# Blosc/c-blosc

Measured on NVIDIA H100. Metric: compress+decompress GB/s, higher is better.
Workload: dtype u8

## Files before the change

c-blosc_b200/csrc/dev_lz4.cuh:

```cuda
#pragma once
#include "dev_common.cuh"

#define LZ4_MFLIMIT 12
#define LZ4_LASTLITERALS 5
#define LZ4_TABLE_BYTES 16384
#define LZ4_TAB17_BYTES (8192 + 512)
#define LZ4_TAB17_MINLEN 65547
#define LZ4_TAB17_MAXLEN 131072

template <bool U16>
DEV u32 lz4_hash_at(const u8* __restrict__ s, int pos) {
  if (U16) return (ld_u32(s + pos) * 2654435761u) >> (32 - 13);
  const u64 seq = (u64)ld_u32(s + pos) | ((u64)s[pos + 4] << 32);
  return (u32)(((seq << 24) * 889523592379ull) >> (64 - 12));
}

#define LZ4_SCALAR_PROBES 4

DEV long long lz4_probe_offset(int it, int accel) {
  if (it == 0) return 0;
  const long long m = it - 1;
  const long long c = m >> 6;
  return 1 + m * accel + 32 * c * (c - 1) + c * (m - 64 * c);
}

struct StreamBase {
  const u8* s;
  const u32* s32;
  int sal;
  const uint4* s128;
  int sal16;
};
DEV StreamBase make_stream_base(const u8* s) {
  StreamBase b;
  b.s = s;
  b.s32 = (const u32*)((uintptr_t)s & ~(uintptr_t)3);
  b.sal = (int)((uintptr_t)s & 3u);
  b.s128 = (const uint4*)((uintptr_t)s & ~(uintptr_t)15);
  b.sal16 = (int)((uintptr_t)s & 15u);
  return b;
}
DEV void ldp_win12(const StreamBase& sb, int p, u32& b0, u32& b1, u32& b2) {
#ifdef SIMT_EMU
  memcpy(&b0, sb.s + p, 4); memcpy(&b1, sb.s + p + 4, 4); memcpy(&b2, sb.s + p + 8, 4);
#else
  const int q = p + sb.sal;
  const u32* w = sb.s32 + (q >> 2);
  const u32 sh = (u32)(q & 3) * 8u;
  const u32 w0 = __ldg(w), w1 = __ldg(w + 1), w2 = __ldg(w + 2), w3 = __ldg(w + 3);
  b0 = __funnelshift_r(w0, w1, sh); b1 = __funnelshift_r(w1, w2, sh); b2 = __funnelshift_r(w2, w3, sh);
#endif
}
DEV void ldp_raw12(const StreamBase& sb, int p, u32& r0, u32& r1, u32& r2, u32& r3) {
#ifdef SIMT_EMU
  memcpy(&r0, sb.s + p, 4); memcpy(&r1, sb.s + p + 4, 4); memcpy(&r2, sb.s + p + 8, 4); r3 = 0;
#else
  const u32* w = sb.s32 + ((p + sb.sal) >> 2);
  r0 = __ldg(w); r1 = __ldg(w + 1); r2 = __ldg(w + 2); r3 = __ldg(w + 3);
#endif
}
DEV void ldp_take12(const StreamBase& sb, int p, u32 r0, u32 r1, u32 r2, u32 r3, u32& b0, u32& b1, u32& b2) {
#ifdef SIMT_EMU
  (void)sb; (void)p; (void)r3; b0 = r0; b1 = r1; b2 = r2;
#else
  const u32 sh = (u32)((p + sb.sal) & 3) * 8u;
  b0 = __funnelshift_r(r0, r1, sh); b1 = __funnelshift_r(r1, r2, sh); b2 = __funnelshift_r(r2, r3, sh);
#endif
}
DEV void ldp_win8(const StreamBase& sb, int p, u32& b0, u32& b1) {
#ifdef SIMT_EMU
  memcpy(&b0, sb.s + p, 4); memcpy(&b1, sb.s + p + 4, 4);
#else
  const int q = p + sb.sal;
  const u32* w = sb.s32 + (q >> 2);
  const u32 sh = (u32)(q & 3) * 8u;
  const u32 w0 = __ldg(w), w1 = __ldg(w + 1), w2 = __ldg(w + 2);
  b0 = __funnelshift_r(w0, w1, sh); b1 = __funnelshift_r(w1, w2, sh);
#endif
}

DEV void ldp_raw20(const StreamBase& sb, int p, u32 (&r)[5]) {
#ifdef SIMT_EMU
  memcpy(&r[0], sb.s + p, 16); r[4] = sb.s[p + 16];
#else
  const u32* w = sb.s32 + ((p + sb.sal) >> 2);
  r[0] = __ldg(w); r[1] = __ldg(w + 1); r[2] = __ldg(w + 2); r[3] = __ldg(w + 3); r[4] = __ldg(w + 4);
#endif
}
DEV void ldp_take17(const StreamBase& sb, int p, const u32 (&r)[5], u32& a0, u32& a1, u32& a2, u32& a3, u32& a4b) {
#ifdef SIMT_EMU
  (void)sb; (void)p; a0 = r[0]; a1 = r[1]; a2 = r[2]; a3 = r[3]; a4b = r[4] & 0xffu;
#else
  const u32 sh = (u32)((p + sb.sal) & 3) * 8u;
  a0 = __funnelshift_r(r[0], r[1], sh); a1 = __funnelshift_r(r[1], r[2], sh);
  a2 = __funnelshift_r(r[2], r[3], sh); a3 = __funnelshift_r(r[3], r[4], sh);
  a4b = (r[4] >> sh) & 0xffu;
#endif
}
DEV void ldp_gather17(const StreamBase& sb, int p, u32& c0, u32& c1, u32& c2, u32& c3, u32& c4b) {
#ifdef SIMT_EMU
  memcpy(&c0, sb.s + p, 4); memcpy(&c1, sb.s + p + 4, 4); memcpy(&c2, sb.s + p + 8, 4); memcpy(&c3, sb.s + p + 12, 4);
  c4b = sb.s[p + 16];
#else
  const int q = p + sb.sal16;
  const uint4* w = sb.s128 + (q >> 4);
  const uint4 v0 = __ldg(w), v1 = __ldg(w + 1);
  const bool k1 = (q & 4) != 0, k2 = (q & 8) != 0;
  const u32 sh = (u32)(q & 3) * 8u;
  const u32 t0 = k1 ? v0.y : v0.x, t1 = k1 ? v0.z : v0.y, t2 = k1 ? v0.w : v0.z, t3 = k1 ? v1.x : v0.w;
  const u32 t4 = k1 ? v1.y : v1.x, t5 = k1 ? v1.z : v1.y, t6 = k1 ? v1.w : v1.z;
  const u32 u0 = k2 ? t2 : t0, u1 = k2 ? t3 : t1, u2 = k2 ? t4 : t2, u3 = k2 ? t5 : t3, u4 = k2 ? t6 : t4;
  c0 = __funnelshift_r(u0, u1, sh); c1 = __funnelshift_r(u1, u2, sh);
  c2 = __funnelshift_r(u2, u3, sh); c3 = __funnelshift_r(u3, u4, sh);
  c4b = (u4 >> sh) & 0xffu;
#endif
}

DEV void lz4d_prefetch(const u8* base, int p, int end) {
#ifndef SIMT_EMU
  if (p < end) asm volatile("prefetch.global.L1 [%0];" :: "l"(base + p));
#else
  (void)base; (void)p; (void)end;
#endif
}

DEV u32 ldp_win4(const StreamBase& sb, int p) {
#ifdef SIMT_EMU
  u32 b0; memcpy(&b0, sb.s + p, 4); return b0;
#else
  const int q = p + sb.sal;
  const u32* w = sb.s32 + (q >> 2);
  return __funnelshift_r(__ldg(w), __ldg(w + 1), (u32)(q & 3) * 8u);
#endif
}

template <bool U16>
DEV u32 lz4_hash_seq(u32 lo, u32 b4) {
  if (U16) return (lo * 2654435761u) >> (32 - 13);
  const u64 seq = (u64)lo | ((u64)(b4 & 0xffu) << 32);
  return (u32)(((seq << 24) * 889523592379ull) >> (64 - 12));
}

DEV int lz4_count_tail(const StreamBase& sb, const u8* __restrict__ s, int p, int q, int limit, int n) {
  if (p + 136 <= n) {
    const int lane = lane_id();
    const u32 x = ldp_win4(sb, p + 4 * lane) ^ ldp_win4(sb, q + 4 * lane);
    const unsigned full = __ballot_sync(FULLMASK, x == 0u);
    if (full != FULLMASK) {
      const int fl = __ffs((int)~full) - 1;
      return fl * 4 + eq_bytes32(__shfl_sync(FULLMASK, x, fl));
    }
    return 128 + warp_count_match(s, p + 128, q + 128, limit);
  }
  return warp_count_match(s, p, q, limit);
}

DEV int lz4_catch_up(const u8* __restrict__ s, int ip, int match, int anchor, int back) {
  const int lane = lane_id();
  for (;;) {
    const int a = ip - 1 - back - lane, b = match - 1 - back - lane;
    const bool ok = a >= anchor && b >= 0 && s[a] == s[b];
    const unsigned m = __ballot_sync(FULLMASK, ok);
    const int step = m == FULLMASK ? 32 : __ffs((int)~m) - 1;
    back += step;
    if (step < 32) return back;
  }
}

#ifdef SIMT_EMU
static long long g_dbg_lz4t_sessions = 0, g_dbg_lz4t_seqs = 0, g_dbg_lz4t_stale = 0, g_dbg_lz4t_x[6];
enum {
  LZ4T_S_HIT0,
  LZ4T_S_STALE = 4,
  LZ4T_S_MISS4,
  LZ4T_S_LIT,
  LZ4T_S_CAPPED,
  LZ4T_S_LONG,
  LZ4T_S_HUGE,
  LZ4T_S_N
};
static long long g_dbg_lz4t_s[LZ4T_S_N];
enum {
  LZ4T_W_WINDOWS,
  LZ4T_W_ELEMS,
  LZ4T_W_STALE0, LZ4T_W_STALEJ,
  LZ4T_W_FWD,
  LZ4T_W_CROSS,
  LZ4T_W_MISS0, LZ4T_W_MISSJ,
  LZ4T_W_LONG0, LZ4T_W_LONGJ,
  LZ4T_W_HUGE,
  LZ4T_W_END, LZ4T_W_CAP, LZ4T_W_TILE,
  LZ4T_W_FULL,
  LZ4T_W_N
};
static long long g_dbg_lz4t_w[LZ4T_W_N];
#define LZ4T_DBG(x) do { if (lane_id() == 0) (x)++; } while (0)
#define LZ4T_DBGN(x, v) do { if (lane_id() == 0) (x) += (v); } while (0)
#else
#define LZ4T_DBG(x) do {} while (0)
#define LZ4T_DBGN(x, v) do {} while (0)
#endif
#ifndef LZ4T_TILES
#define LZ4T_TILES 12
#endif
#ifndef LZ4T_AHEAD
#define LZ4T_AHEAD 8
#endif
#ifndef LZ4T_NAP
#define LZ4T_NAP 128
#endif
#define LZ4T_RING (32 * LZ4T_TILES)
#define LZ4T_BAR_IDLE(i) (1 + (i))
#define LZ4T_BAR_GO(i) (4 + (i))
#define LZ4T_QUIT 1
#define LZ4T_STOP 0x7fffffff
#define LZ4T_END 0xffffffffu
#define LZ4T_LONG 13
#define LZ4T_HSHIFT 19
#define LZ4T_BACKCAP 7
#define LZ4T_W 16
static_assert(LZ4T_TILES % 3 == 0 && LZ4T_AHEAD >= 1 && LZ4T_AHEAD < LZ4T_TILES && LZ4T_RING > 15 + 255 + 4, "team ring layout");
static_assert(2 * LZ4T_W <= 32, "window layout");
#define LZ4T_PREFETCH 512

enum {
  LZ4C_TOTAL,
  LZ4C_START,
  LZ4C_SESSION,
  LZ4C_FULLWAIT,
  LZ4C_REPROBE,
  LZ4C_SEARCH,
  LZ4C_SESSIONS, LZ4C_SEQS, LZ4C_CHAIN_SEQS,
  LZ4C_PREP_BUSY,
  LZ4C_PREP_OWN,
  LZ4C_PREP_GATHER,
  LZ4C_PREP_TILES,
  LZ4C_SMID, LZ4C_SUBP,
  LZ4C_STALE,
  LZ4C_N = 16
};
enum {
  LZ4C_WINDOWS = LZ4C_N, LZ4C_W_STALE, LZ4C_W_MISS, LZ4C_W_LONG, LZ4C_W_END, LZ4C_W_CAP, LZ4C_W_TILE,
  LZ4C_NREC
};
#ifdef B2_LZ4_CYCLES
#define LZ4C_MAXSTREAMS 16384
__device__ unsigned long long g_lz4_cycles[LZ4C_MAXSTREAMS][LZ4C_NREC];
#define LZ4C_T(t) const long long t = clock64()
#define LZ4C_TW(t) const long long t = TEAM ? clock64() : 0ll
#define LZ4C_ADD(k, v) do { if (lane_id() == 0) atomicAdd(&tm->cyc[k], (unsigned long long)(v)); } while (0)
#define LZ4C_SPAN(k, t) LZ4C_ADD(k, clock64() - (t))
#else
#define LZ4C_T(t) do {} while (0)
#define LZ4C_TW(t) do {} while (0)
#define LZ4C_ADD(k, v) do {} while (0)
#define LZ4C_SPAN(k, t) do {} while (0)
#endif

struct Lz4Team {
  uint2 vd[LZ4T_RING];
  int rdy[LZ4T_TILES];
  const u8* s;
  int n;
  int u16;
  int wt;
  int gen;
  int cmd;
  int sub[4];
  int slot;
  u32 seen[8192 / 32];
#ifdef B2_LZ4_CYCLES
  unsigned long long cyc[LZ4C_NREC];
#endif
};
#define LZ4T_SMEM_BYTES ((int)sizeof(Lz4Team))

DEV int lz4t_ld_i32(const int* p) { return *(const volatile int*)p; }
DEV void lz4t_st_i32(int* p, int v) { *(volatile int*)p = v; }

template <bool U16>
DEV void lz4_team_prepare_tile(Lz4Team* tm, const void* tabmem, const u8* s, int n, int tile) {
  const int lane = lane_id();
  const int w0 = 32 * tile, p = w0 + lane;
  const int e = (tile % LZ4T_TILES) * 32 + lane;
  if (w0 + 31 + 24 > n) { tm->vd[e] = make_uint2(0u, LZ4T_END); return; }
  const StreamBase sb = make_stream_base(s);
  u32 r[5], a0, a1, a2, a3, a4, c0, c1, c2, c3, c4;
  LZ4C_T(c_t0);
  ldp_raw20(sb, p, r);
  ldp_take17(sb, p, r, a0, a1, a2, a3, a4);
  const u32 h = lz4_hash_seq<U16>(a0, a1);
  const int snap = U16 ? (int)((const volatile u16*)tabmem)[h] : (int)((const volatile u32*)tabmem)[h];
  u32 vx = h << LZ4T_HSHIFT, sn = LZ4T_END;
  if ((unsigned)snap < (unsigned)p) {
    LZ4C_T(c_t1);
    LZ4C_ADD(LZ4C_PREP_OWN, c_t1 - c_t0);
    ldp_gather17(sb, snap, c0, c1, c2, c3, c4);
    const u32 x1 = a1 ^ c1, x2 = a2 ^ c2, x3 = a3 ^ c3;
    u32 m;
    if (x1) m = (u32)(__ffs((int)x1) - 1) >> 3;
    else if (x2) m = 4u + ((u32)(__ffs((int)x2) - 1) >> 3);
    else if (x3) m = 8u + ((u32)(__ffs((int)x3) - 1) >> 3);
    else m = a4 != c4 ? 12u : (u32)LZ4T_LONG;
    const bool hit = (U16 || snap + 65535 >= p) && c0 == a0;
    u32 bk = 0;
    if (hit) {
      if (snap >= 8) {
        u32 p0, p1, q0, q1;
        ldp_win8(sb, p - 8, p0, p1);
        ldp_win8(sb, snap - 8, q0, q1);
        const u32 y1 = p1 ^ q1, z0 = (u32)__clz((int)(p0 ^ q0)) >> 3;
        bk = y1 ? (u32)__clz((int)y1) >> 3 : 4u + (z0 < 3u ? z0 : 3u);
      } else {
        while (bk < (u32)snap && s[p - 1 - (int)bk] == s[snap - 1 - (int)bk]) bk++;
      }
    }
    vx |= (hit ? 1u : 0u) | (m << 2) | (bk << 8);
    sn = (u32)snap;
    LZ4C_SPAN(LZ4C_PREP_GATHER, c_t1);
  }
  tm->vd[e] = make_uint2(vx, sn);
}

DEV void lz4_team_preparer(Lz4Team* tm, const void* tabmem, int i) {
  for (;;) {
    bar_sync(LZ4T_BAR_GO(i), 64);
    if (lz4t_ld_i32(&tm->cmd) == LZ4T_QUIT) return;
    const u8* s = *(const u8* const volatile*)&tm->s;
    const int n = lz4t_ld_i32(&tm->n), u16 = lz4t_ld_i32(&tm->u16);
    for (int tile = i;; tile += 3) {
      int w;
      for (;;) {
        w = __shfl_sync(FULLMASK, lz4t_ld_i32(&tm->wt), 0);
        if (w == LZ4T_STOP) break;
        if (tile < w) tile = w + (i + 3 - w % 3) % 3;
        if (tile <= w + LZ4T_AHEAD) break;
        __nanosleep(LZ4T_NAP);
      }
      if (w == LZ4T_STOP) break;
      LZ4C_T(c_go);
      lz4d_prefetch(s, 32 * tile + LZ4T_PREFETCH + lane_id(), n);
      if (u16) lz4_team_prepare_tile<true>(tm, tabmem, s, n, tile);
      else lz4_team_prepare_tile<false>(tm, tabmem, s, n, tile);
      __syncwarp();
      if (lane_id() == 0) { __threadfence_block(); lz4t_st_i32(&tm->rdy[tile % LZ4T_TILES], tile + 1); }
      LZ4C_SPAN(LZ4C_PREP_BUSY, c_go);
      LZ4C_ADD(LZ4C_PREP_TILES, 1);
    }
    __syncwarp();
    bar_arrive(LZ4T_BAR_IDLE(i), 64);
  }
}

DEV void lz4t_reach(Lz4Team* tm, int ip, int& wt, int& vt) {
  const int lo = (ip - 2) >> 5, hi = ip >> 5;
  if (lo > wt + LZ4T_AHEAD) LZ4T_DBG(g_dbg_lz4t_x[2]);
  if (lo != wt) { wt = lo; lz4t_st_i32(&tm->wt, lo); }
  for (int t = vt + 1 > lo ? vt + 1 : lo; t <= hi; t++) {
    const int* r = &tm->rdy[t % LZ4T_TILES];
    if (lz4t_ld_i32(r) != t + 1) {
      LZ4T_DBG(g_dbg_lz4t_x[5]);
      do { __syncwarp(); } while (__any_sync(FULLMASK, lz4t_ld_i32(r) != t + 1));
    }
  }
  if (hi > vt) vt = hi;
}

DEV void lz4t_extend(Lz4Team* tm, int wt, int& vt) {
  const int t = vt + 1 + lane_id();
  const bool ready = t <= wt + LZ4T_AHEAD && lz4t_ld_i32(&tm->rdy[t % LZ4T_TILES]) == t + 1;
  vt += __ffs((int)~__ballot_sync(FULLMASK, ready)) - 1;
}

template <bool U16>
DEV bool lz4t_search(Lz4Team* tm, smem_addr_t vda, void* tabmem, const StreamBase& sb, int n, int anchor, int accel,
                     int& twt, int& tvt, u32& pk, u32& snap, int& ip, bool& hit, int& match, int& back, int& lit,
                     bool& have_mc, int& mc_carry) {
  u16* tab16 = (u16*)tabmem;
  u32* tab32 = (u32*)tabmem;
  const int mfl1 = n - LZ4_MFLIMIT + 1;
  ip = anchor + 1;
  int it = 0, pos = ip;
  for (;; it++) {
    if (it == LZ4_SCALAR_PROBES) { LZ4T_DBG(g_dbg_lz4t_s[LZ4T_S_MISS4]); lit = it; return false; }
    pos = ip + (it ? 1 + (it - 1) * accel : 0);
    if (ip + 1 + it * accel > mfl1) { lit = it; return false; }
    if ((pos >> 5) > tvt) lz4t_reach(tm, pos, twt, tvt);
    u32 qk, qs;
    smem_ld_u32x2(vda, ((u32)pos % (u32)LZ4T_RING) << 3, qk, qs);
    const u32 h = qk >> LZ4T_HSHIFT;
    const int cand = U16 ? (int)tab16[h] : (int)tab32[h];
    __syncwarp();
    if (cand != (int)qs) { LZ4T_DBG(g_dbg_lz4t_s[LZ4T_S_STALE]); lit = it; return false; }
    if (U16) tab16[h] = (u16)pos; else tab32[h] = (u32)pos;
    if (qk & 1u) { pk = qk; snap = qs; break; }
  }
  LZ4T_DBG(g_dbg_lz4t_s[LZ4T_S_HIT0 + it]);
  const int vb = (int)((pk >> 8) & 7u), dist = pos - anchor;
  const int bq = vb < dist ? vb : dist;
  int m = (int)((pk >> 2) & 15u);
  if (m == LZ4T_LONG) {
    LZ4T_DBG(g_dbg_lz4t_s[LZ4T_S_LONG]);
    m = LZ4T_LONG + lz4_count_tail(sb, sb.s, pos + 4 + LZ4T_LONG, (int)snap + 4 + LZ4T_LONG, n - LZ4_LASTLITERALS, n);
  }
  if (bq == dist && bq + m < 15 + 255) {
    const int mc = bq + m;
    snap -= (u32)bq;
    pk = 1u | ((u32)(mc < LZ4T_LONG ? mc : LZ4T_LONG) << 2);
    ip = anchor;
    LZ4C_ADD(LZ4C_SEQS, 1);
    LZ4C_ADD(LZ4C_CHAIN_SEQS, ~0ull);
    return true;
  }
  hit = true; ip = pos; match = (int)snap;
  have_mc = true; mc_carry = m;
  back = bq;
  if (vb == LZ4T_BACKCAP && dist > LZ4T_BACKCAP) {
    LZ4T_DBG(g_dbg_lz4t_s[LZ4T_S_CAPPED]);
    back = lz4_catch_up(sb.s, pos, (int)snap, anchor, LZ4T_BACKCAP);
  } else if (bq != dist) LZ4T_DBG(g_dbg_lz4t_s[LZ4T_S_LIT]);
  else LZ4T_DBG(g_dbg_lz4t_s[LZ4T_S_HUGE]);
  lit = pos - back - anchor;
  return false;
}

template <bool U16, bool PACK, bool TEAM>
DEV int lz4_encode_stream(const u8* __restrict__ s, const int n, u8* __restrict__ d, const int cap,
                          const int accel, void* tabmem, int* need_out, Lz4Team* tm) {
  const int lane = lane_id();
  const StreamBase sb = make_stream_base(s);
  u16* tab16 = (u16*)tabmem;
  u32* tab32 = (u32*)tabmem;
  u32* tabhi = (u32*)((u8*)tabmem + 8192);
#define LZ4_TGET(h) (U16 ? (int)tab16[h] : PACK ? ((int)tab16[h] | (int)(((tabhi[(h) >> 5] >> ((h) & 31u)) & 1u) << 16)) : (int)tab32[h])
#define LZ4_TPUT(h, v) do { if (U16) tab16[h] = (u16)(v); else if (PACK) { tab16[h] = (u16)(v); const u32 m_ = 1u << ((h) & 31u); \
                            if ((v) & 0x10000) atomicOr(&tabhi[(h) >> 5], m_); else atomicAnd(&tabhi[(h) >> 5], ~m_); } \
                            else tab32[h] = (u32)(v); } while (0)

  for (int i = lane; i < (PACK ? LZ4_TAB17_BYTES : LZ4_TABLE_BYTES) / 4; i += 32) tab32[i] = 0;
  __syncwarp();

  const bool limited = (long long)cap < (long long)n + n / 255 + 16;
  const int olimit = cap;
  const int mfl1 = n - LZ4_MFLIMIT + 1;
  const int matchlimit = n - LZ4_LASTLITERALS;
  int ip = 1, anchor = 0, op = 0;
  int need = 0;
#define LZ4_LIMIT(v) do { const int v_ = (v); if (v_ > need) need = v_; if (limited && v_ > olimit) return 0; } while (0)

  int w0 = -(1 << 30);
  u32 wq0 = 0, wq1 = 0, wq2 = 0, wh = 0;
  int pb = -(1 << 30);
  u32 pq0 = 0, pq1 = 0, pq2 = 0, pq3 = 0;
  int nrec = 0, recop = 0;
  u32 rec = 0;
  int twt = 0, tvt = -1;
#define LZ4_FLUSH_CHECKED() do { if (nrec) { LZ4_LIMIT(op + (1 + LZ4_LASTLITERALS)); } LZ4_FLUSH(); } while (0)
#define LZ4_FLUSH() do { if (lane < nrec) { d[recop] = (u8)rec; d[recop + 1] = (u8)(rec >> 8); d[recop + 2] = (u8)(rec >> 16); \
                                             if ((rec & 15u) == 15u) d[recop + 3] = (u8)(rec >> 24); } nrec = 0; } while (0)

  if (n >= LZ4_MFLIMIT + 1) {
    bool post = false;
    for (;;) {
      int match = 0, lit = 0, back = 0;
      u32 ipn = 0, cn = 0;
      bool have_next = false, hit = false, imm = false, have_mc = false;
      int mc_carry = 0;

      bool scalar_post = post;
      if constexpr (TEAM) if (post && ip + 64 <= n) {
        scalar_post = false;
        bool finished = false;
        LZ4T_DBG(g_dbg_lz4t_sessions);
        LZ4C_T(c_s0);
        LZ4C_ADD(LZ4C_SESSIONS, 1);
        if ((ip - 2) >> 5 <= twt + LZ4T_AHEAD) LZ4T_DBG(g_dbg_lz4t_x[3]);
        lz4t_reach(tm, ip, twt, tvt);
        __syncwarp();
        LZ4C_SPAN(LZ4C_START, c_s0);
        LZ4C_T(c_s1);
        const smem_addr_t vda = smem_addr(tm->vd);
        u32 e = (u32)ip % (u32)LZ4T_RING;
        bool given = false;
        u32 gpk = 0, gsnap = 0;
        for (;;) {
          if (nrec > 32 - LZ4T_W) {
#ifdef SIMT_EMU
            if (limited && op + 1 + LZ4_LASTLITERALS > olimit) LZ4T_DBG(g_dbg_lz4t_w[LZ4T_W_FULL]);
#endif
            LZ4_FLUSH_CHECKED();
          }
          lz4t_extend(tm, twt, tvt);
          int cnt = 0, q = ip, why;
          u32 ee = e, pk, snap;
          if (given) { pk = gpk; snap = gsnap; } else smem_ld_u32x2(vda, ee << 3, pk, snap);
          int jq = 0;
          u32 je = 0, jpk = 0, jsnap = 0;
          for (;;) {
            if (lane == cnt) { jq = q; je = ee; jpk = pk; jsnap = snap; }
            cnt++;
            const u32 step = ((pk >> 2) & 15u) + 4u;
            u32 en = ee + step;
            if (en >= (u32)LZ4T_RING) en -= (u32)LZ4T_RING;
            u32 npk, nsnap;
            smem_ld_u32x2(vda, en << 3, npk, nsnap);
            if (!(pk & 1u)) { why = LZ4C_W_MISS; break; }
            if (step == LZ4T_LONG + 4u) { why = LZ4C_W_LONG; break; }
            q += (int)step; ee = en;
            if (cnt == LZ4T_W) { why = LZ4C_W_CAP; break; }
            if (q + 64 > n) { why = LZ4C_W_END; break; }
            if ((q >> 5) > tvt) { why = LZ4C_W_TILE; break; }
            pk = npk; snap = nsnap;
          }
          u32 jh2 = 0;
          if (lane < cnt) jh2 = smem_ld_u32(vda, (je >= 2u ? je - 2u : je - 2u + LZ4T_RING) << 3) >> LZ4T_HSHIFT;
          const int el = lane >> 1;
          const bool odd = (lane & 1) != 0;
          const u32 sh2 = __shfl_sync(FULLMASK, jh2, el), sh = __shfl_sync(FULLMASK, jpk >> LZ4T_HSHIFT, el);
          const int sq = __shfl_sync(FULLMASK, jq, el);
          const u32 ssnap = __shfl_sync(FULLMASK, jsnap, el);
          const bool act = lane < 2 * cnt && !(given && lane < 2);
          const u32 skey = odd ? sh : sh2;
          const int spos = odd ? sq : sq - 2;
          int look = 0;
          bool dup = false;
          if (act) {
            if (odd) look = LZ4_TGET(skey);
            const u32 bit = 1u << (skey & 31u);
            dup = (atomicOr(&tm->seen[skey >> 5], bit) & bit) != 0;
          }
          unsigned peers = 1u << lane;
          if (__ballot_sync(FULLMASK, dup)) {
            peers = __match_any_sync(FULLMASK, act ? skey : 0x80000000u | (u32)lane);
            const unsigned lower = peers & ((1u << lane) - 1u);
            const int fpos = __shfl_sync(FULLMASK, spos, lower ? 31 - __clz((int)lower) : lane);
            if (act && odd && lower) look = fpos;
#ifdef SIMT_EMU
            const unsigned fwd = __ballot_sync(FULLMASK, act && odd && lower != 0);
            const unsigned cross = __ballot_sync(FULLMASK, act && !odd && ((peers & 0xaaaaaaaau) & ~(2u << lane)) != 0);
            if (fwd) LZ4T_DBG(g_dbg_lz4t_w[LZ4T_W_FWD]);
            if (cross) LZ4T_DBG(g_dbg_lz4t_w[LZ4T_W_CROSS]);
#endif
          }
          const unsigned bad = __ballot_sync(FULLMASK, act && odd && look != (int)ssnap);
          const int nv = bad ? (__ffs((int)bad) - 1) >> 1 : cnt;
          LZ4T_DBG(g_dbg_lz4t_w[LZ4T_W_WINDOWS]);
          LZ4T_DBGN(g_dbg_lz4t_w[LZ4T_W_ELEMS], nv);
          __syncwarp();
          const unsigned le = nv >= 16 ? FULLMASK : (1u << (2 * nv)) - 1u;
          if (act && lane < 2 * nv && (((peers & le) >> lane) >> 1) == 0) LZ4_TPUT(skey, spos);
          if (act) tm->seen[skey >> 5] = 0u;
          __syncwarp();
          const int nb = nv < cnt || why == LZ4C_W_MISS || why == LZ4C_W_LONG ? (nv < cnt ? nv : cnt - 1) : cnt;
          const u32 rv = (u32)((jpk >> 2) & 15u) | ((u32)(jq - (int)jsnap) << 8);
          const u32 rmine = __shfl_sync(FULLMASK, rv, (lane - nrec) & 31);
          if (lane >= nrec && lane < nrec + nb) { rec = rmine; recop = op + 3 * (lane - nrec); }
          nrec += nb;
          op += 3 * nb;
          LZ4T_DBGN(g_dbg_lz4t_seqs, nb);
          LZ4C_ADD(LZ4C_CHAIN_SEQS, nb);
          LZ4C_ADD(LZ4C_WINDOWS, 1);
          if (nb < cnt) {
            ip = __shfl_sync(FULLMASK, jq, nb);
            e = __shfl_sync(FULLMASK, je, nb);
            snap = __shfl_sync(FULLMASK, jsnap, nb);
          } else { ip = q; e = ee; }
          anchor = ip;
          given = false;
          if (nv < cnt) {
            LZ4T_DBG(g_dbg_lz4t_stale); LZ4C_ADD(LZ4C_STALE, 1); LZ4C_ADD(LZ4C_W_STALE, 1);
            LZ4T_DBG(g_dbg_lz4t_w[nv ? LZ4T_W_STALEJ : LZ4T_W_STALE0]);
            scalar_post = true; break;
          }
          LZ4C_ADD(why, 1);
          if (why == LZ4C_W_MISS) {
            LZ4T_DBG(g_dbg_lz4t_x[4]);
            LZ4T_DBG(g_dbg_lz4t_w[nb ? LZ4T_W_MISSJ : LZ4T_W_MISS0]);
            if (!lz4t_search<U16>(tm, vda, tabmem, sb, n, anchor, accel, twt, tvt, gpk, gsnap, ip, hit, match, back, lit, have_mc, mc_carry))
              break;
            given = true;
            continue;
          }
          if (why == LZ4C_W_LONG) {
            LZ4T_DBG(g_dbg_lz4t_x[0]);
            LZ4T_DBG(g_dbg_lz4t_w[nb ? LZ4T_W_LONGJ : LZ4T_W_LONG0]);
            const int off = ip - (int)snap;
            const int mc = LZ4T_LONG + lz4_count_tail(sb, s, ip + 4 + LZ4T_LONG, ip - off + 4 + LZ4T_LONG, matchlimit, n);
            if (mc >= 15 + 255) {
              hit = true; imm = true; match = ip - off;
              have_mc = true; mc_carry = mc;
              LZ4T_DBG(g_dbg_lz4t_x[1]);
              LZ4T_DBG(g_dbg_lz4t_w[LZ4T_W_HUGE]);
              break;
            }
            const bool ext = mc >= 15;
            LZ4T_DBG(g_dbg_lz4t_seqs);
            LZ4C_ADD(LZ4C_CHAIN_SEQS, 1);
            if (lane == nrec) { rec = (ext ? 15u | ((u32)(mc - 15) << 24) : (u32)mc) | ((u32)off << 8); recop = op; }
            nrec++;
            op += ext ? 4 : 3;
            ip += mc + 4;
            e += (u32)(mc + 4);
            if (e >= (u32)LZ4T_RING) e -= (u32)LZ4T_RING;
            anchor = ip;
          } else if (why == LZ4C_W_CAP) LZ4T_DBG(g_dbg_lz4t_w[LZ4T_W_CAP]);
          else if (why == LZ4C_W_TILE) LZ4T_DBG(g_dbg_lz4t_w[LZ4T_W_TILE]);
          if (ip + 64 > n) {
            if (why == LZ4C_W_END) LZ4T_DBG(g_dbg_lz4t_w[LZ4T_W_END]);
            if (ip >= mfl1) finished = true;
            else scalar_post = true;
            break;
          }
          LZ4C_T(c_w);
          lz4t_reach(tm, ip, twt, tvt);
          LZ4C_SPAN(LZ4C_FULLWAIT, c_w);
        }
        LZ4C_SPAN(LZ4C_SESSION, c_s1);
        if (finished) break;
      }
      if (!TEAM && post && ip + 64 <= n) {
        scalar_post = false;
        bool room = true;
        for (;;) {
          if (ip - 2 < w0 || ip > w0 + 31) {
            if (nrec >= 24) LZ4_FLUSH_CHECKED();
            if (ip - 2 >= pb && ip <= pb + 31) { w0 = pb; ldp_take12(sb, w0 + lane, pq0, pq1, pq2, pq3, wq0, wq1, wq2); }
            else { w0 = ip - 2; ldp_win12(sb, w0 + lane, wq0, wq1, wq2); }
            wh = lz4_hash_seq<U16>(wq0, wq1);
            pb = w0 + 30;
            if (pb + 31 + 16 <= n) ldp_raw12(sb, pb + lane, pq0, pq1, pq2, pq3);
            else pb = -(1 << 30);
            lz4d_prefetch(s, w0 + 192, lane == 0 ? n : 0);
          }
          const int li = ip - w0;
          const u32 h2 = __shfl_sync(FULLMASK, wh, li - 2);
          const u32 h = __shfl_sync(FULLMASK, wh, li);
          const u32 seq = __shfl_sync(FULLMASK, wq0, li);
          const u32 n4 = __shfl_sync(FULLMASK, wq1, li);
          const u32 n8 = __shfl_sync(FULLMASK, wq2, li);
          if (lane == 0) LZ4_TPUT(h2, ip - 2);
          __syncwarp();
          const int cand = LZ4_TGET(h);
          __syncwarp();
          if (lane == 0) LZ4_TPUT(h, ip);
          u32 c0, c1, c2;
          ldp_win12(sb, cand, c0, c1, c2);
          if (!((U16 || cand + 65535 >= ip) && c0 == seq)) { ip++; break; }
          int mc;
          const u32 x1 = n4 ^ c1, x2 = n8 ^ c2;
          if (x1 | x2) {
            const u32 xx = x1 ? x1 : x2;
            mc = ((__ffs((int)xx) - 1) >> 3) + (x1 ? 0 : 4);
          } else {
            u32 p3, p4, q3, q4;
            ldp_win8(sb, ip + 12, p3, p4);
            ldp_win8(sb, cand + 12, q3, q4);
            const u32 x3 = p3 ^ q3, x4 = p4 ^ q4;
            if (x3) mc = 8 + eq_bytes32(x3);
            else if (x4) mc = 12 + eq_bytes32(x4);
            else mc = 16 + lz4_count_tail(sb, s, ip + 20, cand + 20, matchlimit, n);
          }
          if (mc >= 15 + 255) {
            hit = true; imm = true; match = cand;
            have_mc = true; mc_carry = mc;
            break;
          }
          const bool ext = mc >= 15;
          const int off = ip - cand;
          if (lane == nrec) { rec = (ext ? 15u | ((u32)(mc - 15) << 24) : (u32)mc) | ((u32)off << 8); recop = op; }
          nrec++;
          op += ext ? 4 : 3;
          ip += mc + 4;
          anchor = ip;
          if (ip + 64 > n) { room = false; break; }
        }
        if (!room) {
          if (ip >= mfl1) break;
          continue;
        }
      }
      if (scalar_post) {
        LZ4C_TW(c_r);
        u32 b0, b1, b2 = 0;
        const bool wide = ip + 14 <= n;
        if (wide) ldp_win12(sb, ip - 2, b0, b1, b2);
        else { b0 = ld_u32(s + ip - 2); b1 = ld_u32(s + ip + 2); }
        const u32 seq = __funnelshift_r(b0, b1, 16);
        const u32 h2 = lz4_hash_seq<U16>(b0, b1);
        const u32 h = lz4_hash_seq<U16>(seq, b1 >> 16);
        if (lane == 0) LZ4_TPUT(h2, ip - 2);
        __syncwarp();
        const int cand = LZ4_TGET(h);
        __syncwarp();
        if (lane == 0) LZ4_TPUT(h, ip);
        if (U16 || cand + 65535 >= ip) {
          u32 c0, c1;
          ldp_win8(sb, cand, c0, c1);
          if (c0 == seq) {
            hit = true; imm = true; match = cand;
            ipn = __funnelshift_r(b1, b2, 16); cn = c1; have_next = wide;
          }
        }
        if (!hit) ip++;
        if (TEAM) LZ4C_SPAN(LZ4C_REPROBE, c_r);
      }

      if (!hit) {
        LZ4C_TW(c_f);
        bool ended = false;
        for (int it = TEAM ? lit : 0; it < LZ4_SCALAR_PROBES; it++) {
          const int pos = ip + (it ? 1 + (it - 1) * accel : 0);
          if (ip + 1 + it * accel > mfl1) { ended = true; break; }
          u32 b0, b1 = 0, b2 = 0;
          const bool wide = pos + 16 <= n;
          if (wide) ldp_win12(sb, pos, b0, b1, b2);
          else { b0 = ld_u32(s + pos); b1 = (u32)s[pos + 4]; }
          const u32 h = lz4_hash_seq<U16>(b0, b1);
          __syncwarp();
          const int cand = LZ4_TGET(h);
          __syncwarp();
          if (lane == 0) LZ4_TPUT(h, pos);
          if (U16 || cand + 65535 >= pos) {
            u32 c0, c1;
            ldp_win8(sb, cand, c0, c1);
            if (c0 == b0) {
              hit = true; ip = pos; match = cand;
              ipn = b1; cn = c1; have_next = wide;
              break;
            }
          }
        }
        if (!hit && !ended) {
          __syncwarp();
          for (int base_it = LZ4_SCALAR_PROBES;; base_it += 32) {
            const int itl = base_it + lane;
            const bool valid = ip + lz4_probe_offset(itl + 1, accel) <= mfl1;
            const int pos = valid ? ip + (int)lz4_probe_offset(itl, accel) : 0;
            u32 h = 0x80000000u | (u32)lane, seq = 0;
            if (valid) { seq = ld_u32(s + pos); h = lz4_hash_at<U16>(s, pos); }
            const unsigned vmask = __ballot_sync(FULLMASK, valid);
            const unsigned peers = __match_any_sync(FULLMASK, h);
            const unsigned lower = peers & ((1u << lane) - 1u);
            int cand = 0;
            bool lhit = false;
            if (valid) {
              cand = lower ? ip + (int)lz4_probe_offset(base_it + (31 - __clz((int)lower)), accel) : LZ4_TGET(h);
              if (U16 || cand + 65535 >= pos) lhit = ld_u32(s + cand) == seq;
            }
            const unsigned found = __ballot_sync(FULLMASK, lhit);
            const int nvalid = __popc(vmask);
            const int f = found ? __ffs((int)found) - 1 : 32;
            const int last = f < nvalid - 1 ? f : nvalid - 1;
            __syncwarp();
            if (valid && lane <= last) {
              const unsigned le = last >= 31 ? FULLMASK : ((1u << (last + 1)) - 1u);
              if ((((peers & le) >> lane) >> 1) == 0) LZ4_TPUT(h, pos);
            }
            __syncwarp();
            if (found) {
              ip = __shfl_sync(FULLMASK, pos, f);
              match = __shfl_sync(FULLMASK, cand, f);
              hit = true;
              break;
            }
            if (nvalid < 32) break;
          }
        }
        if (!hit) { if (TEAM) LZ4C_SPAN(LZ4C_SEARCH, c_f); break; }

        if (ip > anchor && match > 0 && s[ip - 1] == s[match - 1]) back = lz4_catch_up(s, ip, match, anchor, 0);
        lit = ip - back - anchor;
        if (TEAM) LZ4C_SPAN(LZ4C_SEARCH, c_f);
      }

      int mc;
      if (have_mc) mc = mc_carry;
      else {
        const int room = matchlimit - (ip + 4);
        if (have_next) {
          const u32 x = ipn ^ cn;
          if (x) mc = eq_bytes32(x);
          else if (room > 20) {
            u32 p0, p1, p2, q0, q1, q2;
            ldp_win12(sb, ip + 8, p0, p1, p2);
            ldp_win12(sb, match + 8, q0, q1, q2);
            const u32 x0 = p0 ^ q0, x1 = p1 ^ q1, x2 = p2 ^ q2;
            if (x0) mc = 4 + eq_bytes32(x0);
            else if (x1) mc = 8 + eq_bytes32(x1);
            else if (x2) mc = 12 + eq_bytes32(x2);
            else mc = 16 + lz4_count_tail(sb, s, ip + 20, match + 20, matchlimit, n);
          } else mc = 4 + (room > 4 ? warp_count_match(s, ip + 8, match + 8, matchlimit) : 0);
          if (mc > room) mc = room;
        } else mc = warp_count_match(s, ip + 4, match + 4, matchlimit);
      }
      const int off = ip - match;
      ip += mc + 4;
      mc += back;

      if (TEAM) LZ4C_ADD(LZ4C_SEQS, 1);
      LZ4_FLUSH_CHECKED();
      const int token = op++;
      if (!imm) LZ4_LIMIT(op + lit + (2 + 1 + LZ4_LASTLITERALS) + lit / 255);
      if (lit < 15 && mc < 15) {
        LZ4_LIMIT(op + lit + 2 + (1 + LZ4_LASTLITERALS));
        u32 v;
        if (lane == 0) v = ((u32)lit << 4) | (u32)mc;
        else if (lane <= lit) v = s[anchor + lane - 1];
        else v = lane == lit + 1 ? (u32)off : (u32)off >> 8;
        if (lane <= lit + 2) d[token + lane] = (u8)v;
        op += lit + 2;
      } else {
        u32 tokval;
        if (lit >= 15) {
          const int len = lit - 15, nff = len / 255;
          tokval = 15u << 4;
          warp_fill_bytes(d + op, nff, 255);
          if (lane == 0) d[op + nff] = (u8)(len - nff * 255);
          op += nff + 1;
        } else tokval = (u32)lit << 4;
        warp_copy_bytes(d + op, s + anchor, lit);
        op += lit;
        if (lane == 0) { d[op] = (u8)off; d[op + 1] = (u8)(off >> 8); }
        op += 2;
        LZ4_LIMIT(op + (1 + LZ4_LASTLITERALS) + (mc + 240) / 255);
        if (mc >= 15) {
          tokval += 15;
          const int rest = mc - 15, nff = rest / 255;
          warp_fill_bytes(d + op, nff, 255);
          if (lane == 0) d[op + nff] = (u8)(rest - nff * 255);
          op += nff + 1;
        } else tokval += (u32)mc;
        if (lane == 0) d[token] = (u8)tokval;
      }

      anchor = ip;
      if (ip >= mfl1) break;
      post = true;
    }
  }

  LZ4_FLUSH_CHECKED();
  const int lastRun = n - anchor;
  LZ4_LIMIT(op + lastRun + 1 + (lastRun + 255 - 15) / 255);
  if (lastRun >= 15) {
    const int acc = lastRun - 15, nff = acc / 255;
    if (lane == 0) d[op] = (u8)(15u << 4);
    op++;
    warp_fill_bytes(d + op, nff, 255);
    if (lane == 0) d[op + nff] = (u8)(acc - nff * 255);
    op += nff + 1;
  } else {
    if (lane == 0) d[op] = (u8)(lastRun << 4);
    op++;
  }
  warp_copy_bytes(d + op, s + anchor, lastRun);
  op += lastRun;
  *need_out = need;
  return op;
#undef LZ4_FLUSH_CHECKED
#undef LZ4_FLUSH
#undef LZ4_LIMIT
#undef LZ4_TGET
#undef LZ4_TPUT
}

DEV void lz4t_begin(Lz4Team* tm, const u8* s, int n, bool u16) {
  const int lane = lane_id();
  for (int i = lane; i < LZ4T_TILES; i += 32) tm->rdy[i] = 0;
  for (int i = lane; i < 8192 / 32; i += 32) tm->seen[i] = 0;
  if (lane == 0) { tm->s = s; tm->n = n; tm->u16 = u16 ? 1 : 0; tm->wt = 0; tm->gen = tm->gen + 1; }
  __syncwarp();
  __threadfence_block();
  bar_arrive(LZ4T_BAR_GO(0), 64); bar_arrive(LZ4T_BAR_GO(1), 64); bar_arrive(LZ4T_BAR_GO(2), 64);
}
DEV void lz4t_end(Lz4Team* tm) {
  __syncwarp();
  if (lane_id() == 0) lz4t_st_i32(&tm->wt, LZ4T_STOP);
// ... 422 lines not shown
```

Baseline: 127.8.

## Widen preparer loads to include back bytes and prefetch next tile's window

The preparer warp now loads a 28-byte window covering 8 bytes before each position, and the gather loads 8 extra bytes before the candidate. The separate backward-extension loads and the scalar loop for small offsets go away, and the backward length is taken from the widened registers and clamped to the snap offset. It also issues the raw loads for the tile three steps ahead before doing the current tile's gather, software-pipelining global latency across tiles. Extra cycle-counter slots are added for instrumentation only. The costs are more registers and extra loads for tiles that never hit.

```diff
diff --git a/c-blosc_b200/csrc/dev_lz4.cuh b/c-blosc_b200/csrc/dev_lz4.cuh
--- a/c-blosc_b200/csrc/dev_lz4.cuh
+++ b/c-blosc_b200/csrc/dev_lz4.cuh
@@ -79,40 +79,49 @@
 #endif
 }
 
-DEV void ldp_raw20(const StreamBase& sb, int p, u32 (&r)[5]) {
+DEV void ldp_raw28(const StreamBase& sb, int p, u32 (&r)[7]) {
 #ifdef SIMT_EMU
-  memcpy(&r[0], sb.s + p, 16); r[4] = sb.s[p + 16];
+  const int back = p < 8 ? p : 8;
+  r[0] = r[1] = 0u;
+  memcpy((u8*)r + 8 - back, sb.s + p - back, back); memcpy(&r[2], sb.s + p, 16); r[6] = sb.s[p + 16];
 #else
-  const u32* w = sb.s32 + ((p + sb.sal) >> 2);
-  r[0] = __ldg(w); r[1] = __ldg(w + 1); r[2] = __ldg(w + 2); r[3] = __ldg(w + 3); r[4] = __ldg(w + 4);
-#endif
-}
-DEV void ldp_take17(const StreamBase& sb, int p, const u32 (&r)[5], u32& a0, u32& a1, u32& a2, u32& a3, u32& a4b) {
+  const int wi = ((p + sb.sal) >> 2) - 2;
+  const u32* w = sb.s32 + wi;
+  r[0] = wi >= 0 ? __ldg(w) : 0u; r[1] = wi >= -1 ? __ldg(w + 1) : 0u;
+  r[2] = __ldg(w + 2); r[3] = __ldg(w + 3); r[4] = __ldg(w + 4); r[5] = __ldg(w + 5); r[6] = __ldg(w + 6);
+#endif
+}
+DEV void ldp_take25(const StreamBase& sb, int p, const u32 (&r)[7], u32 (&b)[7]) {
 #ifdef SIMT_EMU
-  (void)sb; (void)p; a0 = r[0]; a1 = r[1]; a2 = r[2]; a3 = r[3]; a4b = r[4] & 0xffu;
+  (void)sb; (void)p; for (int k = 0; k < 6; k++) b[k] = r[k]; b[6] = r[6] & 0xffu;
 #else
   const u32 sh = (u32)((p + sb.sal) & 3) * 8u;
-  a0 = __funnelshift_r(r[0], r[1], sh); a1 = __funnelshift_r(r[1], r[2], sh);
-  a2 = __funnelshift_r(r[2], r[3], sh); a3 = __funnelshift_r(r[3], r[4], sh);
-  a4b = (r[4] >> sh) & 0xffu;
-#endif
-}
-DEV void ldp_gather17(const StreamBase& sb, int p, u32& c0, u32& c1, u32& c2, u32& c3, u32& c4b) {
+#pragma unroll
+  for (int k = 0; k < 6; k++) b[k] = __funnelshift_r(r[k], r[k + 1], sh);
+  b[6] = (r[6] >> sh) & 0xffu;
+#endif
+}
+DEV void ldp_gather25(const StreamBase& sb, int p, u32 (&c)[7]) {
 #ifdef SIMT_EMU
-  memcpy(&c0, sb.s + p, 4); memcpy(&c1, sb.s + p + 4, 4); memcpy(&c2, sb.s + p + 8, 4); memcpy(&c3, sb.s + p + 12, 4);
-  c4b = sb.s[p + 16];
+  const int back = p < 8 ? p : 8;
+  c[0] = c[1] = 0u;
+  memcpy((u8*)c + 8 - back, sb.s + p - back, back); memcpy(&c[2], sb.s + p, 16); c[6] = sb.s[p + 16];
 #else
   const int q = p + sb.sal16;
   const uint4* w = sb.s128 + (q >> 4);
+  const uint2 vm = q >= 16 ? __ldg((const uint2*)w - 1) : make_uint2(0u, 0u);
   const uint4 v0 = __ldg(w), v1 = __ldg(w + 1);
   const bool k1 = (q & 4) != 0, k2 = (q & 8) != 0;
   const u32 sh = (u32)(q & 3) * 8u;
-  const u32 t0 = k1 ? v0.y : v0.x, t1 = k1 ? v0.z : v0.y, t2 = k1 ? v0.w : v0.z, t3 = k1 ? v1.x : v0.w;
-  const u32 t4 = k1 ? v1.y : v1.x, t5 = k1 ? v1.z : v1.y, t6 = k1 ? v1.w : v1.z;
+  const u32 t0 = k1 ? vm.y : vm.x, t1 = k1 ? v0.x : vm.y, t2 = k1 ? v0.y : v0.x, t3 = k1 ? v0.z : v0.y;
+  const u32 t4 = k1 ? v0.w : v0.z, t5 = k1 ? v1.x : v0.w, t6 = k1 ? v1.y : v1.x, t7 = k1 ? v1.z : v1.y;
+  const u32 t8 = k1 ? v1.w : v1.z;
   const u32 u0 = k2 ? t2 : t0, u1 = k2 ? t3 : t1, u2 = k2 ? t4 : t2, u3 = k2 ? t5 : t3, u4 = k2 ? t6 : t4;
-  c0 = __funnelshift_r(u0, u1, sh); c1 = __funnelshift_r(u1, u2, sh);
-  c2 = __funnelshift_r(u2, u3, sh); c3 = __funnelshift_r(u3, u4, sh);
-  c4b = (u4 >> sh) & 0xffu;
+  const u32 u5 = k2 ? t7 : t5, u6 = k2 ? t8 : t6;
+  c[0] = __funnelshift_r(u0, u1, sh); c[1] = __funnelshift_r(u1, u2, sh);
+  c[2] = __funnelshift_r(u2, u3, sh); c[3] = __funnelshift_r(u3, u4, sh);
+  c[4] = __funnelshift_r(u4, u5, sh); c[5] = __funnelshift_r(u5, u6, sh);
+  c[6] = (u6 >> sh) & 0xffu;
 #endif
 }
 
@@ -221,7 +230,9 @@
 #define LZ4T_W 16
 static_assert(LZ4T_TILES % 3 == 0 && LZ4T_AHEAD >= 1 && LZ4T_AHEAD < LZ4T_TILES && LZ4T_RING > 15 + 255 + 4, "team ring layout");
 static_assert(2 * LZ4T_W <= 32, "window layout");
+#ifndef LZ4T_PREFETCH
 #define LZ4T_PREFETCH 512
+#endif
 
 enum {
   LZ4C_TOTAL,
@@ -241,6 +252,9 @@
 };
 enum {
   LZ4C_WINDOWS = LZ4C_N, LZ4C_W_STALE, LZ4C_W_MISS, LZ4C_W_LONG, LZ4C_W_END, LZ4C_W_CAP, LZ4C_W_TILE,
+  LZ4C_W_TILE_LEAD,
+  LZ4C_W_TILE_JUMP,
+  LZ4C_PREP_WAIT,
   LZ4C_NREC
 };
 #ifdef B2_LZ4_CYCLES
@@ -250,11 +264,15 @@
 #define LZ4C_TW(t) const long long t = TEAM ? clock64() : 0ll
 #define LZ4C_ADD(k, v) do { if (lane_id() == 0) atomicAdd(&tm->cyc[k], (unsigned long long)(v)); } while (0)
 #define LZ4C_SPAN(k, t) LZ4C_ADD(k, clock64() - (t))
+#define LZ4C_VAR(v, x) long long v = (x)
+#define LZ4C_SET(v, x) v = (x)
 #else
 #define LZ4C_T(t) do {} while (0)
 #define LZ4C_TW(t) do {} while (0)
 #define LZ4C_ADD(k, v) do {} while (0)
 #define LZ4C_SPAN(k, t) do {} while (0)
+#define LZ4C_VAR(v, x) do {} while (0)
+#define LZ4C_SET(v, x) do {} while (0)
 #endif
 
 struct Lz4Team {
@@ -279,43 +297,34 @@
 DEV void lz4t_st_i32(int* p, int v) { *(volatile int*)p = v; }
 
 template <bool U16>
-DEV void lz4_team_prepare_tile(Lz4Team* tm, const void* tabmem, const u8* s, int n, int tile) {
+DEV void lz4_team_prepare_tile(Lz4Team* tm, const void* tabmem, const StreamBase& sb, int n, int tile, u32 (&r)[7], int& nt) {
   const int lane = lane_id();
   const int w0 = 32 * tile, p = w0 + lane;
   const int e = (tile % LZ4T_TILES) * 32 + lane;
-  if (w0 + 31 + 24 > n) { tm->vd[e] = make_uint2(0u, LZ4T_END); return; }
-  const StreamBase sb = make_stream_base(s);
-  u32 r[5], a0, a1, a2, a3, a4, c0, c1, c2, c3, c4;
+  if (w0 + 31 + 24 > n) { tm->vd[e] = make_uint2(0u, LZ4T_END); nt = -1; return; }
   LZ4C_T(c_t0);
-  ldp_raw20(sb, p, r);
-  ldp_take17(sb, p, r, a0, a1, a2, a3, a4);
-  const u32 h = lz4_hash_seq<U16>(a0, a1);
+  if (nt != tile) ldp_raw28(sb, p, r);
+  u32 a[7], c[7];
+  ldp_take25(sb, p, r, a);
+  const u32 h = lz4_hash_seq<U16>(a[2], a[3]);
   const int snap = U16 ? (int)((const volatile u16*)tabmem)[h] : (int)((const volatile u32*)tabmem)[h];
+  nt = w0 + 96 + 31 + 24 > n ? -1 : tile + 3;
+  if (nt >= 0) ldp_raw28(sb, p + 96, r);
   u32 vx = h << LZ4T_HSHIFT, sn = LZ4T_END;
   if ((unsigned)snap < (unsigned)p) {
     LZ4C_T(c_t1);
     LZ4C_ADD(LZ4C_PREP_OWN, c_t1 - c_t0);
-    ldp_gather17(sb, snap, c0, c1, c2, c3, c4);
-    const u32 x1 = a1 ^ c1, x2 = a2 ^ c2, x3 = a3 ^ c3;
+    ldp_gather25(sb, snap, c);
+    const u32 x1 = a[3] ^ c[3], x2 = a[4] ^ c[4], x3 = a[5] ^ c[5];
     u32 m;
     if (x1) m = (u32)(__ffs((int)x1) - 1) >> 3;
     else if (x2) m = 4u + ((u32)(__ffs((int)x2) - 1) >> 3);
     else if (x3) m = 8u + ((u32)(__ffs((int)x3) - 1) >> 3);
-    else m = a4 != c4 ? 12u : (u32)LZ4T_LONG;
-    const bool hit = (U16 || snap + 65535 >= p) && c0 == a0;
-    u32 bk = 0;
-    if (hit) {
-      if (snap >= 8) {
-        u32 p0, p1, q0, q1;
-        ldp_win8(sb, p - 8, p0, p1);
-        ldp_win8(sb, snap - 8, q0, q1);
-        const u32 y1 = p1 ^ q1, z0 = (u32)__clz((int)(p0 ^ q0)) >> 3;
-        bk = y1 ? (u32)__clz((int)y1) >> 3 : 4u + (z0 < 3u ? z0 : 3u);
-      } else {
-        while (bk < (u32)snap && s[p - 1 - (int)bk] == s[snap - 1 - (int)bk]) bk++;
-      }
-    }
-    vx |= (hit ? 1u : 0u) | (m << 2) | (bk << 8);
+    else m = a[6] != c[6] ? 12u : (u32)LZ4T_LONG;
+    const bool hit = (U16 || snap + 65535 >= p) && c[2] == a[2];
+    const u32 y1 = a[1] ^ c[1], z0 = (u32)__clz((int)(a[0] ^ c[0])) >> 3;
+    const u32 bk = min(y1 ? (u32)__clz((int)y1) >> 3 : 4u + min(z0, 3u), (u32)snap);
+    vx |= hit ? 1u | (m << 2) | (bk << 8) : m << 2;
     sn = (u32)snap;
     LZ4C_SPAN(LZ4C_PREP_GATHER, c_t1);
   }
@@ -328,8 +337,12 @@
     if (lz4t_ld_i32(&tm->cmd) == LZ4T_QUIT) return;
     const u8* s = *(const u8* const volatile*)&tm->s;
     const int n = lz4t_ld_i32(&tm->n), u16 = lz4t_ld_i32(&tm->u16);
+    const StreamBase sb = make_stream_base(s);
+    u32 r[7];
+    int nt = -1;
     for (int tile = i;; tile += 3) {
       int w;
+      LZ4C_T(c_wait);
       for (;;) {
         w = __shfl_sync(FULLMASK, lz4t_ld_i32(&tm->wt), 0);
         if (w == LZ4T_STOP) break;
@@ -337,11 +350,12 @@
         if (tile <= w + LZ4T_AHEAD) break;
         __nanosleep(LZ4T_NAP);
       }
+      LZ4C_SPAN(LZ4C_PREP_WAIT, c_wait);
       if (w == LZ4T_STOP) break;
       LZ4C_T(c_go);
       lz4d_prefetch(s, 32 * tile + LZ4T_PREFETCH + lane_id(), n);
-      if (u16) lz4_team_prepare_tile<true>(tm, tabmem, s, n, tile);
-      else lz4_team_prepare_tile<false>(tm, tabmem, s, n, tile);
+      if (u16) lz4_team_prepare_tile<true>(tm, tabmem, sb, n, tile, r, nt);
+      else lz4_team_prepare_tile<false>(tm, tabmem, sb, n, tile, r, nt);
       __syncwarp();
       if (lane_id() == 0) { __threadfence_block(); lz4t_st_i32(&tm->rdy[tile % LZ4T_TILES], tile + 1); }
       LZ4C_SPAN(LZ4C_PREP_BUSY, c_go);
@@ -483,6 +497,7 @@
         u32 e = (u32)ip % (u32)LZ4T_RING;
         bool given = false;
         u32 gpk = 0, gsnap = 0;
+        LZ4C_VAR(c_steady, 0);
         for (;;) {
           if (nrec > 32 - LZ4T_W) {
 #ifdef SIMT_EMU
@@ -491,6 +506,7 @@
             LZ4_FLUSH_CHECKED();
           }
           lz4t_extend(tm, twt, tvt);
+          LZ4C_VAR(c_lead, tvt - (ip >> 5));
           int cnt = 0, q = ip, why;
           u32 ee = e, pk, snap;
           if (given) { pk = gpk; snap = gsnap; } else smem_ld_u32x2(vda, ee << 3, pk, snap);
@@ -573,6 +589,10 @@
             scalar_post = true; break;
           }
           LZ4C_ADD(why, 1);
+#ifdef B2_LZ4_CYCLES
+          if (why == LZ4C_W_TILE) { LZ4C_ADD(LZ4C_W_TILE_LEAD, c_lead); LZ4C_ADD(LZ4C_W_TILE_JUMP, !c_steady); }
+#endif
+          LZ4C_SET(c_steady, why == LZ4C_W_CAP || why == LZ4C_W_TILE);
           if (why == LZ4C_W_MISS) {
             LZ4T_DBG(g_dbg_lz4t_x[4]);
             LZ4T_DBG(g_dbg_lz4t_w[nb ? LZ4T_W_MISSJ : LZ4T_W_MISS0]);
```

Result: no change. 128.8 (median of 6 runs) (+0.8%).
